# vani-nag/OWLRayTracing

Hardware: AMD Instinct MI355X
Metric: kNN queries/sec (10M pts, k=10) (higher is better)
Workload: dtype f32; 1 GPU; TrueKNN on 10000000 uniform-random 3-D points (numpy default_rng(0), [0,1)^3), k=10, start radius 0.25*(k/n)^(1/3)=0.0025; BASELINE.json configs[1]; ranks=1, n_points_total=10000000, k=10, kernel=team_kernel, parallelism=1 GPU

## Files before the change

### owlraytracing_amd/csrc/team_args.h

```cpp
#pragma once
#include <stdint.h>

#include <algorithm>
#include <cstdlib>

#include "lbvh.h"
#include "owlknn.h"

#ifndef TKNN_DIAG_BUILD
#define TKNN_DIAG_BUILD 0
#endif

namespace owlmi {

constexpr int kTeamBlock = 64;
inline int grab_for(int64_t count, int blocks, int turns, int cap) {
  if (const char *g = getenv("TKNN_GRAB")) return std::max(1, atoi(g));
  return (int)std::max<int64_t>(1, std::min<int64_t>(cap, count / ((int64_t)std::max(1, blocks) * 4 * turns)));
}
#ifndef TKNN_NREG3
#define TKNN_NREG3 1
#endif
inline int nreg_for(int k) { return k <= 16 ? 1 : (k <= 32 ? 2 : (k <= 48 && TKNN_NREG3 ? 3 : 4)); }

struct TeamArgs {
  LbvhView bvh, halo;
  LbvhWideView wide[2];
  float start_radius;
  const float *start_radii;
  int k;
  int max_rounds;
  int allow_unfinished;
  int first_step;
  int first_ext;
  float tie_span;
  int diag;
  int32_t ngroups;
  int32_t *out_idx;
  float *out_dist;
  int64_t *out_isect;
  tknnNeigh *out_fb;
  int32_t *out_level;
  uint8_t *done;
  int64_t *isect_sorted;
  int32_t *next_level;
  uint8_t *tie;
  int32_t *tie_list;
  const uint8_t *skip;
  int32_t skip_is;
  const int32_t *slot_count;
  int grab;
  const int32_t *row_slot;
  unsigned long long *counters;
};

}
```

### owlraytracing_amd/csrc/trueknn_team.hip

```cpp
#include "knn_thresholds.h"
#include "team_args.h"
#include "team_lanes.h"
#include "team_walk.h"
#include "trueknn_engine.h"

#include <algorithm>
#include <cmath>
#include <cstdio>
#include <cstdlib>
#include <cstring>

namespace owlmi {

namespace {

#ifndef TKNN_MAX_BLOCKS_3
#define TKNN_MAX_BLOCKS_3 256
#endif
#ifndef TKNN_MAX_BLOCKS_4
#define TKNN_MAX_BLOCKS_4 512
#endif
constexpr int max_blocks(int nreg) { return nreg == 4 ? TKNN_MAX_BLOCKS_4 : (nreg == 3 ? TKNN_MAX_BLOCKS_3 : 256); }
#ifndef TKNN_MAX_PER_QUERY
#define TKNN_MAX_PER_QUERY 72
#endif
#ifndef TKNN_MAX_PER_QUERY_2
#define TKNN_MAX_PER_QUERY_2 88
#endif
#ifndef TKNN_MAX_PER_QUERY_3
#define TKNN_MAX_PER_QUERY_3 88
#endif
#ifndef TKNN_MAX_PER_QUERY_4
#define TKNN_MAX_PER_QUERY_4 124
#endif
constexpr int max_per_query(int nreg) {
  return nreg == 1 ? TKNN_MAX_PER_QUERY : (nreg == 4 ? TKNN_MAX_PER_QUERY_4 : (nreg == 3 ? TKNN_MAX_PER_QUERY_3 : TKNN_MAX_PER_QUERY_2));
}
inline int lds_workgroups_per_cu(size_t lds) {
  const size_t granule = 1280, total = 160 * 1024;
  return lds ? (int)((total / granule) / ((lds + granule - 1) / granule)) : 1 << 20;
}
#ifndef TKNN_SORT_FIRST
#define TKNN_SORT_FIRST 1
#endif
#ifndef TKNN_TEAM_WAVES
#define TKNN_TEAM_WAVES 4
#endif
constexpr int kXcdCounter = kDbStats, kXcdCounterStride = 32;
constexpr int kTeamStack = 192;
constexpr int kQrecStride = 6;
constexpr int kScanBudget = 16384;
constexpr int kMaxStep = 2;
constexpr int kLdsQrec = 64 * kQrecStride * 4;
constexpr int kLdsCnt = 64 * 2 * 4;
constexpr int kLdsList = 64 * 4 + 16;
constexpr int kLdsStack = kTeamStack * 4;
constexpr int kLdsShared = (kLdsCnt + kLdsList) > kLdsStack ? (kLdsCnt + kLdsList) : kLdsStack;
constexpr int kLdsSharedPadded = (kLdsShared + 15) & ~15;
constexpr int kCandCap = kCandCapacity;
template <int NREG>
struct TeamLayout {
  static constexpr int kMaxPerQuery = max_per_query(NREG);
  static constexpr int kMaxBlocks = max_blocks(NREG);
  static constexpr int kLdsBlk = kMaxBlocks * 4;
  static constexpr int kLdsMask = 64 * kMaxPerQuery;
  static constexpr int kHiWords = kMaxBlocks > 256 ? (kMaxPerQuery + 31) / 32 : 0;
  static constexpr int kLdsHi = 64 * kHiWords * 4;
  static constexpr int kEntStride = kMaxPerQuery + 4;
  static constexpr int kLdsEnt = 4 * kEntStride * 4;
  static constexpr int kLdsCand = 4 * kCandCap * 8;
  static constexpr int kOffMask = kLdsQrec + kLdsBlk;
  static constexpr int kOffHi = kOffMask + kLdsMask;
  static constexpr int kOffShared = kOffHi + kLdsHi;
  static constexpr int kOffEnt = kOffShared + kLdsSharedPadded;
  static constexpr int kOffCand = kOffEnt + kLdsEnt;
  static constexpr int kTeamLds = kOffCand + kLdsCand;
  static_assert(kEntStride % 4 == 0 && kOffEnt % 16 == 0, "entry lists must be 16-byte aligned");
  static_assert(kLdsMask % 4 == 0, "the ninth bits are words");
  static_assert(kMaxPerQuery <= 124 && kMaxPerQuery / 4 < 32, "list-length buckets of the pass lists are one bit each of a 32-bit word");
};

struct TeamLds {
  float *qrec;
  int32_t *blk;
  uint8_t *qblk;
  uint32_t *qhi;
  uint32_t *qcnt;
  int32_t *qlist;
  int32_t *ent;
  unsigned long long *cand;
};

template <bool SELECT, bool HALO, int NREG, bool FULL, bool TWO>
__device__ __forceinline__ void team_pass(const TeamArgs &a, const TeamLds &L, int n_list, int32_t first_slot,
                                          const LbvhPoint *own_pts, const LbvhPoint *halo_pts, int lane) {
  const int team = lane >> 4, tl = lane & 15;
  constexpr int kMaxPerQuery = TeamLayout<NREG>::kMaxPerQuery, kEntStride = TeamLayout<NREG>::kEntStride;
  static_assert(!(SELECT && TWO), "only a COUNT pass serves two levels");
  n_list = __builtin_amdgcn_readfirstlane(n_list);
  [[maybe_unused]] unsigned long long tp[4] = {0, 0, 0, 0};
  for (int r0 = 0; r0 < n_list; r0 += 4) {
    [[maybe_unused]] unsigned long long tp_mark = 0;
    if (TKNN_DIAG_BUILD && (a.diag & 128)) tp_mark = __builtin_amdgcn_s_memtime();
#define TP_LAP(i)                                                     \
  do {                                                                \
    if (TKNN_DIAG_BUILD && (a.diag & 128)) {                          \
      const unsigned long long now_ = __builtin_amdgcn_s_memtime();   \
      tp[i] += now_ - tp_mark;                                        \
      tp_mark = now_;                                                 \
    }                                                                 \
  } while (0)
    const bool on = r0 + team < n_list;
    int qi = 0;
    if (on) qi = L.qlist[r0 + team];
    const float *rec = L.qrec + qi * kQrecStride;
    const float t_qx = rec[0], t_qy = rec[1], t_qz = rec[2];
    const int32_t t_qid = __float_as_int(rec[3]);
    const float t_r = rec[4];
    const float t_mg = (fmaxf(fmaxf(fabsf(t_qx), fabsf(t_qy)), fabsf(t_qz)) + 2.0f * t_r) * 4.76837158203125e-07f;
    const float in_below = t_r - t_mg, in_upto = t_r + t_mg;
    const float r_inner = t_r * 0.5f;
    const float i0_below = r_inner - t_mg, i0_upto = r_inner + t_mg;
    uint32_t cnt_i0 = 0;
    const int packed = __float_as_int(rec[5]);
    [[maybe_unused]] int32_t out_row = 0;
    if (SELECT) out_row = a.bvh.prim_id[first_slot + qi];
    const int my_n = on ? (packed & 0xff) : 0;
    const int steps = max(max((int)__builtin_amdgcn_readlane(my_n, 0), (int)__builtin_amdgcn_readlane(my_n, 16)),
                          max((int)__builtin_amdgcn_readlane(my_n, 32), (int)__builtin_amdgcn_readlane(my_n, 48)));
    if (TKNN_DIAG_BUILD && (a.diag & 16) && lane == 0) atomicAdd(&a.counters[15], (unsigned long long)steps);
    const uint8_t *mine = L.qblk + qi * kMaxPerQuery;
    const int last = my_n - 1;
    const int32_t nan_block = a.wide[0].count[0];
    const int own_pos = (packed >> 8) & 0xff;
    const int n_near = (packed >> 16) & 0xff;
    const int last_near = n_near ? n_near - 1 : last;
    const int both = min(own_pos, last_near - own_pos);
    const bool right_longer = last_near - own_pos > own_pos;
    auto list_pos = [&](int it) -> int {
      if (!SELECT) return it;
      const int half = (it + 1) >> 1;
      const int alt = (it & 1) ? half : -half;
      const int far = it - both;
      const int off = it <= 2 * both ? alt : (right_longer ? far : -far);
      return it > last_near ? it : own_pos + off;
    };
    auto list_entry = [&](int pos) -> int32_t {
      int lp = list_pos(pos);
      if (n_near && lp >= n_near) lp = kMaxPerQuery - 1 - (lp - n_near);
      const int at = min(max(lp, 0), kMaxPerQuery - 1);
      int slot_at = mine[at];
      if (TeamLayout<NREG>::kHiWords) slot_at |= (int)((L.qhi[qi * TeamLayout<NREG>::kHiWords + (at >> 5)] >> (at & 31)) & 1u) << 8;
      int32_t e = L.blk[slot_at];
      if (TKNN_DIAG_BUILD && (a.diag & 64)) e = L.blk[mine[0]];
      return resolve_entry<HALO>(pos <= last ? e : nan_block);
    };
    const int steps4 = (steps + 3) & ~3;
    int32_t *my_ent = L.ent + team * kEntStride;
    for (int base = 0; base < steps4 + 4; base += 16)
      if (base + tl < kEntStride) my_ent[base + tl] = list_entry(base + tl);
    t_wave_sync();
    uint32_t cnt = 0;
    uint32_t bd[NREG], bi[NREG];
#pragma unroll
    for (int j = 0; j < NREG; j++) {
      bd[j] = 0x7f7fffffu;
      bi[j] = 0u;
    }
    constexpr bool full = FULL;
    uint32_t left_out = 0xffffffffu;
    auto kth_dist = [&]() -> float {
      uint32_t reg = bd[0];
#pragma unroll
      for (int j = 1; j < NREG; j++) reg = ((a.k - 1) >> 4) == j ? bd[j] : reg;
      return __uint_as_float(t_lane_read(reg, (team << 4) + ((a.k - 1) & 15)));
    };
    float tau2 = INFINITY;
    bool dirty = false;
    uint32_t fill_n = 0;
    auto merge_buffer = [&]() {
      t_wave_sync();
      t_merge_rows<NREG>(bd, bi, left_out, full, L.cand + team * kCandCap, fill_n, tl);
      t_wave_sync();
      fill_n = 0;
      dirty = false;
      tau2 = knn_gate_from_worst(kth_dist());
    };
    auto in_box = [&](const LbvhPoint &p, float t, float radius, float below, float upto) -> unsigned long long {
      unsigned long long in_m = __ballot(t <= below);
      const unsigned long long maybe = __ballot(t <= upto);
      if (__builtin_expect(maybe != in_m, 0)) in_m |= maybe & __ballot(knn_in_box(p.x, p.y, p.z, radius, t_qx, t_qy, t_qz));
      return in_m;
    };
    auto process = [&](const LbvhPoint &p, bool own_block = false) {
      const float dx = p.x - t_qx, dy = p.y - t_qy, dz = p.z - t_qz;
      const float t = fmaxf(fmaxf(fabsf(dx), fabsf(dy)), fabsf(dz));
      const unsigned long long in_m = in_box(p, t, t_r, in_below, in_upto);
      cnt = t_count_keep(cnt, in_m, p.id);
      if (TWO) cnt_i0 = t_count(cnt_i0, in_box(p, t, r_inner, i0_below, i0_upto));
      if (SELECT) {
        const float d2 = t_dist2(dx, dy, dz);
        unsigned long long pm = in_m & __ballot(d2 <= tau2);
        if (own_block) pm &= __ballot(p.id != t_qid);
        if (TKNN_DIAG_BUILD && (a.diag & 1)) pm = 0;
        if (pm) {
          if (TKNN_DIAG_BUILD && (a.diag & 16) && lane == 0) atomicAdd(&a.counters[26], (unsigned long long)__popcll(pm));
          const uint32_t mine16 = (uint32_t)(pm >> (team << 4)) & 0xffffu;
          if ((mine16 >> tl) & 1u) {
            const unsigned long long key = ((unsigned long long)__float_as_uint(d2) << 32) | (uint32_t)p.id;
            L.cand[team * kCandCap + fill_n + __popc(mine16 & ((1u << tl) - 1u))] = key;
          }
          fill_n += __popc(mine16);
          dirty = true;
          if (__ballot(fill_n >= 16u) != 0ull) {
            if (TKNN_DIAG_BUILD && (a.diag & 16) && lane == 0) atomicAdd(&a.counters[27], 1ull);
            merge_buffer();
          }
        }
      }
    };
    const LbvhPoint *own_base = a.bvh.points;
    const uint32_t lane_bytes = (uint32_t)tl * (uint32_t)sizeof(LbvhPoint);
    typedef int32_t t_int4 __attribute__((ext_vector_type(4)));
    const t_int4 *my_groups = (const t_int4 *)my_ent;
    auto fetch = [&](int32_t entry) -> t_point4 {
      const LbvhPoint p = load_block_point<HALO>(own_pts, halo_pts, entry, own_base, lane_bytes);
      return t_point4{p.x, p.y, p.z, __int_as_float(p.id)};
    };
    auto unpack = [](const t_point4 &v) -> LbvhPoint { return LbvhPoint{v.x, v.y, v.z, __float_as_int(v.w)}; };
    auto sort_first = [&](const LbvhPoint &p) {
      const float dx = p.x - t_qx, dy = p.y - t_qy, dz = p.z - t_qz;
      const float t = fmaxf(fmaxf(fabsf(dx), fabsf(dy)), fabsf(dz));
      bool in = t <= t_r;
      if (__ballot(fabsf(t - t_r) <= t_mg) != 0ull) in = (t <= in_below) || ((t <= in_upto) && knn_in_box(p.x, p.y, p.z, t_r, t_qx, t_qy, t_qz));
      cnt = t_count(cnt, __ballot(in));
      bool cand = in && (p.id != t_qid);
      if (TKNN_DIAG_BUILD && (a.diag & 1)) cand = false;
      const uint32_t d2_bits = __float_as_uint(t_dist2(dx, dy, dz));
      unsigned long long *my_buf = L.cand + team * kCandCap;
      my_buf[tl] = ((unsigned long long)d2_bits << 32) | (uint32_t)p.id;
      t_wave_sync();
      t_sorted_row(d2_bits, (uint32_t)p.id, cand, tl, [&](int from) { return my_buf[from]; }, bd[0], bi[0]);
      t_wave_sync();
      tau2 = knn_gate_from_worst(kth_dist());
    };
    TP_LAP(0);
    t_point4 b0, b1, b2, b3;
    {
      const t_int4 g = my_groups[0];
      b0 = fetch(g.x);
      __builtin_amdgcn_sched_barrier(0);
      b1 = fetch(g.y);
      __builtin_amdgcn_sched_barrier(0);
      b2 = fetch(g.z);
      __builtin_amdgcn_sched_barrier(0);
      b3 = fetch(g.w);
      __builtin_amdgcn_sched_barrier(0);
    }
    for (int it = 0; it < steps; it += 4) {
      const t_int4 g = my_groups[(it >> 2) + 1];
      if (SELECT && it == 0) {
        if (NREG == 1 && TKNN_SORT_FIRST == 0)
          process(unpack(b0), true);
        else
          sort_first(unpack(b0));
      } else {
        process(unpack(b0));
      }
      b0 = fetch(g.x);
      process(unpack(b1));
      b1 = fetch(g.y);
      process(unpack(b2));
      b2 = fetch(g.z);
      process(unpack(b3));
      b3 = fetch(g.w);
      if (SELECT && dirty && __ballot(fill_n >= (uint32_t)TKNN_MERGE_AT) != 0ull) {
        if (TKNN_DIAG_BUILD && (a.diag & 16) && lane == 0) atomicAdd(&a.counters[27], 1ull);
        merge_buffer();
      }
      TP_LAP(it == 0 ? 1 : 2);
    }
    if (SELECT && dirty) {
      if (TKNN_DIAG_BUILD && (a.diag & 16) && lane == 0) atomicAdd(&a.counters[27], 1ull);
      merge_buffer();
    }
    if (SELECT && full) {
      uint32_t v = left_out;
      v = min(v, (uint32_t)__builtin_amdgcn_update_dpp(-1, (int)v, 0x128 , 0xf, 0xf, false));
      v = min(v, (uint32_t)__builtin_amdgcn_update_dpp(-1, (int)v, 0x124 , 0xf, 0xf, false));
      v = min(v, (uint32_t)__builtin_amdgcn_update_dpp(-1, (int)v, 0x122 , 0xf, 0xf, false));
      v = min(v, (uint32_t)__builtin_amdgcn_update_dpp(-1, (int)v, 0x121 , 0xf, 0xf, false));
      left_out = v;
    }
    cnt = t_team_sum(cnt);
    const uint32_t self = cnt ? 1u : 0u;
    const uint32_t others = cnt - self;
    if (TWO) cnt_i0 = t_team_sum(cnt_i0);
    uint32_t tied = 0u;
    if (SELECT) {
      bool tie[NREG];
      bool any = false;
#pragma unroll
      for (int j = 0; j < NREG; j++) {
        uint32_t before = t_team_shr1(bd[j]);
        if (j > 0) before |= t_dpp<0x121>(bd[j - 1]) & (tl == 0 ? 0xffffffffu : 0u);
        tie[j] = ((j > 0) | (tl >= 1)) & (16 * j + tl <= a.k) & (bd[j] == before);
        if (full && j == NREG - 1) tie[j] |= (tl == 15) & (left_out == bd[j]);
        any |= tie[j];
      }
      if (__ballot(any) != 0ull) {
        const float qmax = fmaxf(fmaxf(fabsf(t_qx), fabsf(t_qy)), fabsf(t_qz));
        any = false;
        bool edge = false;
        const float q_r0 = a.start_radii ? a.start_radii[a.bvh.prim_id[first_slot + qi]] : a.start_radius;
#pragma unroll
        for (int j = 0; j < NREG; j++) {
          const bool t = tie[j] && tie_may_straddle(__uint_as_float(bd[j]), q_r0, t_r, qmax, a.tie_span);
          any |= t;
          edge |= t && (16 * j + tl == a.k || (full && j == NREG - 1 && tl == 15 && left_out == bd[j]));
        }
        if (on && edge) knn_note_tie_edge(a.tie, first_slot + qi);
      }
      tied = ((uint32_t)(__ballot(any) >> (team * 16)) & 0xffffu) ? 1u : 0u;
    }
    if (on && tl == 0) {
      uint32_t *out = L.qcnt + qi * 2;
      if (!TWO) {
        out[0] = cnt;
        out[1] = (self << 31) | (tied << 30);
      } else {
        out[0] = cnt_i0;
        out[1] = cnt | (self << 31);
      }
    }
    if (SELECT) {
      if (on && others >= (uint32_t)a.k) {
#pragma unroll
        for (int reg = 0; reg < NREG; reg++) {
          const int j = tl + 16 * reg;
          if (j >= a.k) continue;
          const int64_t o = (int64_t)out_row * a.k + j;
          const int32_t prim = knn_key_prim(((uint64_t)bd[reg] << 32) | bi[reg]);
          const float d = __uint_as_float(bd[reg]);
          if (a.out_idx) a.out_idx[o] = prim;
          if (a.out_dist) a.out_dist[o] = d;
          if (a.out_fb) {
            int2 *rec8 = (int2 *)(a.out_fb + o);
            rec8[0] = make_int2(prim, __float_as_int(d));
            rec8[1] = make_int2(j == 0 ? 0 : a.k, 0);
            if (j != 0) rec8[2] = make_int2(0, 0);
          }
        }
      }
    }
    TP_LAP(3);
  }
#undef TP_LAP
  if (TKNN_DIAG_BUILD && (a.diag & 128) && lane == 0)
    for (int i = 0; i < 4; i++) atomicAdd(&a.counters[(SELECT ? 36 : 28) + i], tp[i]);
}

template <bool HALO, int NREG, bool FULL>
__global__ void __launch_bounds__(kTeamBlock) __attribute__((amdgpu_waves_per_eu(TKNN_TEAM_WAVES))) team_kernel(TeamArgs a) {
  extern __shared__ __align__(16) unsigned char smem[];
  const int lane = threadIdx.x & 63;
  const int wid = threadIdx.x >> 6;
  const int tl = lane & 15;
  using Lay = TeamLayout<NREG>;
  constexpr int kMaxPerQuery = Lay::kMaxPerQuery;
  unsigned char *base = smem + wid * Lay::kTeamLds;
  float *qrec = (float *)base;
  int32_t *blk = (int32_t *)(base + kLdsQrec);
  uint8_t *qblk = (uint8_t *)(base + Lay::kOffMask);
  uint32_t *qhi = (uint32_t *)(base + Lay::kOffHi);
  constexpr int kMaxBlocks = Lay::kMaxBlocks;
  uint32_t *qcnt = (uint32_t *)(base + Lay::kOffShared);
  int32_t *qlist = (int32_t *)(base + Lay::kOffShared + kLdsCnt);
  int32_t *stack = (int32_t *)(base + Lay::kOffShared);
  int32_t *ent = (int32_t *)(base + Lay::kOffEnt);
  unsigned long long *cand = (unsigned long long *)(base + Lay::kOffCand);

  const LbvhPoint *own_pts = a.bvh.points + tl, *halo_pts = a.halo.points ? a.halo.points + tl : a.bvh.points + tl;
  unsigned long long my_isect_sum = 0, wave_node_tests = 0, wave_point_tests = 0;
  uint32_t my_levels = 0, my_unfinished = 0;
  int wave_levels = 0, wave_err = 0;
  uint32_t my_handed = 0;
  [[maybe_unused]] unsigned long long diag_scanned = 0, diag_listed = 0;
  int wave_min_handover = 0x7fffffff;
#if TKNN_DIAG_BUILD
  unsigned long long ph[5] = {0, 0, 0, 0, 0}, t_mark = __builtin_amdgcn_s_memtime();
#define PHASE_END(i)                                         \
  do {                                                       \
    const unsigned long long now_ = __builtin_amdgcn_s_memtime(); \
    ph[i] += now_ - t_mark;                                  \
    t_mark = now_;                                           \
  } while (0)
#else
#define PHASE_END(i) \
  do {               \
  } while (0)
#endif

  const int xcc = (int)__builtin_amdgcn_s_getreg(6164 ) & 7;
  const int chunk = max(1, min(1024, a.ngroups / 128));
  uint32_t seg_empty = 0;
  for (;;) {
    int g = -1;
    for (int t = 0; t < 8 && g < 0; t++) {
      const int x = (xcc + t) & 7;
      if (seg_empty & (1u << x)) continue;
      int v = 0;
      if (lane == 0) v = (int)atomicAdd(&a.counters[kXcdCounter + kXcdCounterStride * x], 1ull);
      v = __builtin_amdgcn_readfirstlane(v);
      const int cand = ((v / chunk) * 8 + x) * chunk + (v % chunk);
      if (cand < a.ngroups)
        g = cand;
      else
        seg_empty |= 1u << x;
    }
    if (g < 0 || wave_err) break;

    const int32_t slot = g * 64 + lane;
    bool active = slot < a.bvh.n;
    if (a.skip) {
      if (active && (int32_t)a.skip[slot] == a.skip_is) active = false;
      if (__ballot(active) == 0ull) continue;
    }
    LbvhPoint q = {0.f, 0.f, 0.f, -1};
    if (active) q = a.bvh.points[slot];
    const int32_t row = active ? a.bvh.prim_id[slot] : 0;
    float r = a.start_radius;
    if (a.start_radii && active) r = a.start_radii[row];
    int level = 0;
    int64_t isect = 0;
    uint32_t prev_others = 0;
    int step = a.first_step;
    TeamLds L;
    L.qrec = qrec;
    L.blk = blk;
    L.qblk = qblk;
    L.qhi = qhi;
    L.qcnt = qcnt;
    L.qlist = qlist;
    L.ent = ent;
    L.cand = cand;

    bool reuse = false;
    int ext_next = a.first_ext;
    bool ext_ok = a.first_ext >= 0;
    for (;;) {
      PHASE_END(4);
      level = __builtin_amdgcn_readfirstlane(level);
      step = __builtin_amdgcn_readfirstlane(step);
      if (!a.start_radii) r = __uint_as_float(__builtin_amdgcn_readfirstlane(__float_as_uint(r)));
      int m = step < 1 ? 1 : (step > kMaxStep ? kMaxStep : step);
      if (reuse) m = 1;
      if (level + m > a.max_rounds) m = a.max_rounds - level;
      const float r_in0 = r;
      float r_out = r;
      for (int j = 1; j < m; j++) r_out = r_out * 2.0f;
      {
        float *rec = qrec + lane * kQrecStride;
        rec[0] = q.x;
        rec[1] = q.y;
        rec[2] = q.z;
        rec[3] = __int_as_float(q.id);
        rec[4] = r_out;
      }
      int my_nblk = 0;
      int n_in = 0, n_out = 0;
      int my_own_pos = 0;
      bool too_big = false;
      bool ext = !reuse && ext_next > 0 && level + m < a.max_rounds;
      ext = __builtin_amdgcn_readfirstlane((int)ext) != 0;
      if (reuse) {
        const int pk = __float_as_int(qrec[lane * kQrecStride + 5]);
        n_in = pk & 0xff;
        my_own_pos = (pk >> 8) & 0xff;
        n_out = (pk >> 24) & 0xff;
        my_nblk = n_in + n_out;
        reuse = false;
      } else
      for (;;) {
      const float r_walk = ext ? r_out * 2.0f : r_out;
      float lo_x = INFINITY, lo_y = INFINITY, lo_z = INFINITY, hi_x = -INFINITY, hi_y = -INFINITY, hi_z = -INFINITY;
      float reach_walk = -INFINITY, reach_step = -INFINITY;
      {
        const float qabs = fmaxf(fmaxf(fabsf(q.x), fabsf(q.y)), fabsf(q.z));
        const float mg = (qabs + 2.0f * r_walk) * 4.76837158203125e-07f;
        if (active && q.x == q.x) {
          lo_x = (q.x - r_walk) - 2.0f * mg;
          lo_y = (q.y - r_walk) - 2.0f * mg;
          lo_z = (q.z - r_walk) - 2.0f * mg;
          hi_x = (q.x + r_walk) + 2.0f * mg;
          hi_y = (q.y + r_walk) + 2.0f * mg;
          hi_z = (q.z + r_walk) + 2.0f * mg;
          reach_walk = r_walk + 2.0f * mg;
          reach_step = ext ? r_out + 2.0f * ((qabs + 2.0f * r_out) * 4.76837158203125e-07f) : reach_walk;
        }
      }
      float s_lo_x[4], s_lo_y[4], s_lo_z[4], s_hi_x[4], s_hi_y[4], s_hi_z[4];
      {
        const float r_lo_x = t_team_min(lo_x), r_lo_y = t_team_min(lo_y), r_lo_z = t_team_min(lo_z);
        const float r_hi_x = t_team_max(hi_x), r_hi_y = t_team_max(hi_y), r_hi_z = t_team_max(hi_z);
#pragma unroll
        for (int j = 0; j < 4; j++) {
          s_lo_x[j] = t_bcast(r_lo_x, 16 * j);
          s_lo_y[j] = t_bcast(r_lo_y, 16 * j);
          s_lo_z[j] = t_bcast(r_lo_z, 16 * j);
          s_hi_x[j] = t_bcast(r_hi_x, 16 * j);
          s_hi_y[j] = t_bcast(r_hi_y, 16 * j);
          s_hi_z[j] = t_bcast(r_hi_z, 16 * j);
        }
      }
      auto separation = [](float b_lo_x, float b_lo_y, float b_lo_z, float b_hi_x, float b_hi_y, float b_hi_z, float q_lo_x, float q_lo_y,
                           float q_lo_z, float q_hi_x, float q_hi_y, float q_hi_z) -> float {
        const float sx = fmaxf(b_lo_x - q_hi_x, q_lo_x - b_hi_x), sy = fmaxf(b_lo_y - q_hi_y, q_lo_y - b_hi_y),
                    sz = fmaxf(b_lo_z - q_hi_z, q_lo_z - b_hi_z);
        return fmaxf(fmaxf(sx, sy), sz);
      };
      auto overlaps_packet = [&](const LbvhBox &bx) -> bool {
        float best = INFINITY;
#pragma unroll
        for (int j = 0; j < 4; j++)
          best = fminf(best, separation(bx.lo[0], bx.lo[1], bx.lo[2], bx.hi[0], bx.hi[1], bx.hi[2], s_lo_x[j], s_lo_y[j], s_lo_z[j], s_hi_x[j],
                                        s_hi_y[j], s_hi_z[j]));
        return best <= 0.f;
      };
      float *node_boxes = (float *)ent;
      static_assert(64 * 6 * 4 <= Lay::kLdsEnt + Lay::kLdsCand, "the gather's child boxes borrow the entry lists' LDS");
      auto stash_boxes = [&](const LbvhBox &bx) {
        float2 *dst = (float2 *)(node_boxes + 6 * lane);
        dst[0] = make_float2(bx.lo[0], bx.lo[1]);
        dst[1] = make_float2(bx.lo[2], bx.hi[0]);
        dst[2] = make_float2(bx.hi[1], bx.hi[2]);
        t_wave_sync();
      };
      auto gap_to_me = [&](int src) -> float {
        int boff;
        asm("s_mul_i32 %0, %1, 24" : "=s"(boff) : "s"(src));
        const float2 *b = (const float2 *)((const char *)node_boxes + boff);
        const float2 b0 = b[0], b1 = b[1], b2 = b[2];
        return separation(b0.x, b0.y, b1.x, b1.y, b2.x, b2.y, q.x, q.y, q.z, q.x, q.y, q.z);
      };

      PHASE_END(0);
      my_own_pos = 0;
      int cur = 0;
      uint8_t *my_list = qblk + lane * kMaxPerQuery;
      if (Lay::kHiWords) {
#pragma unroll
        for (int w = 0; w < Lay::kHiWords; w++) qhi[lane * Lay::kHiWords + w] = 0u;
      }
      int nb = 0, scanned = 0;
      for (int tree = 0; tree < 2 && !too_big; tree++) {
        const LbvhWideView &wv = a.wide[tree];
        const int32_t tree_n = tree == 0 ? a.bvh.n : a.halo.n;
        if (tree_n <= 0 || wv.levels <= 0) continue;
        int sp = 0, nleaf = 0;
        if (lane == 0) stack[wv.levels > 1 ? 0 : kTeamStack - 1] = (wv.levels << 26) | 0;
        if (wv.levels > 1)
          sp = 1;
        else
          nleaf = 1;
        t_wave_sync();
        const int32_t last_block = wv.count[0] - 1;
        while ((sp > 0 || nleaf > 0) && !too_big) {
          if (sp > 0 && sp + nleaf + 63 <= kTeamStack) {
            const int32_t e = __builtin_amdgcn_readfirstlane(stack[sp - 1]);
            sp--;
            const int lvl = (e >> 26) - 1;
            const int32_t first_child = (e & 0x3ffffff) * 64;
            const int32_t c = first_child + lane;
            const bool valid = lvl == wv.levels - 1 ? (lane < wv.count[lvl] && first_child == 0) : (c < wv.count[lvl]);
            LbvhBox bx = {{0.f, 0.f, 0.f}, {0.f, 0.f, 0.f}};
            if (valid) bx = wv.level[lvl][c];
            wave_node_tests += 64;
            const bool ov = valid & overlaps_packet(bx);
            const unsigned long long om = __ballot(ov);
            const int cnt = __popcll(om);
            if (lvl > 1) {
              if (ov) stack[sp + t_rank(om)] = (lvl << 26) | c;
              sp += cnt;
            } else {
              unsigned long long rest = om;
              if (rest) stash_boxes(bx);
              while (rest) {
                const int src = 63 - __builtin_clzll(rest);
                rest &= ~(1ull << src);
                if (__ballot(gap_to_me(src) <= reach_walk) == 0ull) continue;
                if (lane == 0) stack[kTeamStack - 1 - nleaf] = (lvl << 26) | (first_child + src);
                nleaf++;
              }
            }
            t_wave_sync();
            continue;
          }
          if (nleaf == 0) {
            too_big = true;
            break;
          }
          auto leaf_boxes = [&](int i) -> LbvhBox {
            const int32_t e = __builtin_amdgcn_readfirstlane(stack[kTeamStack - nleaf + (i < nleaf ? i : nleaf - 1)]);
            return wv.level[0][min((e & 0x3ffffff) * 64 + lane, last_block)];
          };
          LbvhBox bx_next = leaf_boxes(0);
          for (int i = 0; i < nleaf && !too_big; i++) {
            const int32_t e = __builtin_amdgcn_readfirstlane(stack[kTeamStack - nleaf + i]);
            const int32_t first_child = (e & 0x3ffffff) * 64;
            const LbvhBox bx = bx_next;
            bx_next = leaf_boxes(i + 1);
            const bool valid = first_child + lane <= last_block;
            wave_node_tests += 64;
            const bool ov = valid & overlaps_packet(bx);
            unsigned long long om = __ballot(ov);
            scanned += __popcll(om);
            if (TKNN_DIAG_BUILD && (a.diag & 32)) diag_scanned += __popcll(om);
            if (scanned > kScanBudget) {
              too_big = true;
              break;
            }
            if (om) stash_boxes(bx);
            while (om) {
              const int src = __ffsll((long long)om) - 1;
              om &= om - 1;
              const float gap = gap_to_me(src);
              bool need = gap <= reach_walk;
              if (TKNN_DIAG_BUILD && (a.diag & 8)) need = false;
              if (__ballot(need) == 0ull) continue;
              if (nb >= kMaxBlocks) {
                too_big = true;
                break;
              }
              const int32_t block = first_child + src;
              blk[nb] = (int32_t)((uint32_t)block | ((uint32_t)tree << 31));
              if (tree == 0 && (uint32_t)(block - g * 4) < 4u && block == (slot >> 4)) my_own_pos = cur & 0xffff;
              if (need) {
                const bool inner = gap <= reach_step;
                const int at = inner ? (cur & 0xffff) : kMaxPerQuery - 1 - (cur >> 16);
                const int at_c = min(max(at, 0), kMaxPerQuery - 1);
                my_list[at_c] = (uint8_t)nb;
                if (Lay::kHiWords && nb >= 256) qhi[lane * Lay::kHiWords + (at_c >> 5)] |= 1u << (at_c & 31);
                cur += inner ? 1 : 0x10000;
              }
              nb++;
            }
          }
          nleaf = 0;
          t_wave_sync();
        }
        t_wave_sync();
      }
      if (TKNN_DIAG_BUILD && (a.diag & 32)) diag_listed += nb;
      n_in = cur & 0xffff, n_out = cur >> 16;
      if (ext) {
        if (too_big || __ballot(n_in + n_out > kMaxPerQuery) != 0ull) {
          ext = false;
          ext_ok = false;
          too_big = false;
          t_wave_sync();
          continue;
        }
        reuse = __ballot(active) != 0ull;
      }
      my_nblk = n_in;
      if (!ext) n_out = 0;
      break;
      }
      if (NREG < 3) {
        if (__ballot(my_nblk > kMaxPerQuery) != 0ull) too_big = true;
        if (too_big) {
          if (active) {
            a.done[slot] = 0;
            a.isect_sorted[slot] = isect;
            a.next_level[slot] = level;
            my_handed++;
          }
          wave_min_handover = min(wave_min_handover, level);
          active = false;
          break;
        }
      } else if (too_big || __ballot(my_nblk > kMaxPerQuery) != 0ull) {
        const bool hand_over = active && (too_big || my_nblk > kMaxPerQuery);
        if (hand_over) {
          a.done[slot] = 0;
          a.isect_sorted[slot] = isect;
          a.next_level[slot] = level;
          my_handed++;
          active = false;
        }
        wave_min_handover = min(wave_min_handover, level);
        if (__ballot(active) == 0ull) break;
      }
      const int my_packed = my_nblk | (my_own_pos << 8) | (my_nblk > n_in ? n_in << 16 : n_out << 24);
      qrec[lane * kQrecStride + 5] = __int_as_float(my_packed);

      PHASE_END(1);
      const bool speculate = m == 1 && active && level > 0 && prev_others * 8u >= (uint32_t)(a.k + a.k / 2);
      const bool count_first = active && !speculate;
      auto build_qlist = [&](bool sel) -> int {
        const int bucket = my_nblk >> 2;
        if (lane == 0) qlist[64] = 0;
        t_wave_sync();
        if (sel) __hip_atomic_fetch_or((uint32_t *)&qlist[64], 1u << bucket, __ATOMIC_RELAXED, __HIP_MEMORY_SCOPE_WAVEFRONT);
        t_wave_sync();
        uint32_t present = (uint32_t)__builtin_amdgcn_readfirstlane(qlist[64]);
        int base = 0, pos = 0;
        while (present) {
          const int b = __ffs((int)present) - 1;
          present &= present - 1u;
          const bool mine = sel && bucket == b;
          const unsigned long long bm = __ballot(mine);
          if (mine) pos = base + t_rank(bm);
          base += __popcll(bm);
        }
        if (sel) qlist[pos] = lane;
        t_wave_sync();
        return base;
      };
      {
        const int n_count = build_qlist(count_first);
        if (!(TKNN_DIAG_BUILD && (a.diag & 4))) {
          if (m > 1)
            team_pass<false, HALO, NREG, false, true>(a, L, n_count, g * 64, own_pts, halo_pts, lane);
          else
            team_pass<false, HALO, NREG, false, false>(a, L, n_count, g * 64, own_pts, halo_pts, lane);
        }
        t_wave_sync();
      }
      PHASE_END(2);
      uint32_t c0 = 0, c1 = 0, selfc = 0;
      int fin_at = -1;
      if (count_first) {
        c0 = qcnt[lane * 2 + 0];
        const uint32_t w1 = qcnt[lane * 2 + 1];
        c1 = m > 1 ? (w1 & 0x3fffffffu) : 0u;
        selfc = w1 >> 31;
        if (c0 - selfc >= (uint32_t)a.k)
          fin_at = 0;
        else if (m > 1 && c1 - selfc >= (uint32_t)a.k)
          fin_at = 1;
      }
      const bool select_now = speculate || fin_at >= 0;
      if (m > 1 && fin_at == 0) qrec[lane * kQrecStride + 4] = r_in0;
      {
        t_wave_sync();
        const int n_select = build_qlist(select_now);
        if (!(TKNN_DIAG_BUILD && (a.diag & 2))) team_pass<true, HALO, NREG, FULL, false>(a, L, n_select, g * 64, own_pts, halo_pts, lane);
        t_wave_sync();
      }
      PHASE_END(3);
      bool finished = fin_at >= 0;
      uint32_t last_others = 0;
      if (speculate) {
        c0 = qcnt[lane * 2 + 0];
        selfc = qcnt[lane * 2 + 1] >> 31;
        finished = c0 - selfc >= (uint32_t)a.k;
        fin_at = finished ? 0 : -1;
      }
      int levels_run = 0;
      if (active) {
        levels_run = finished ? fin_at + 1 : m;
        isect += c0;
        if (levels_run > 1) isect += c1;
        my_levels += (uint32_t)levels_run;
        last_others = (m > 1 ? c1 : c0) - selfc;
        prev_others = last_others;
      }
      wave_levels = max(wave_levels, (int)t_wave_max((float)(active ? level + levels_run : 0)));
      {
        const unsigned long long passes = (count_first ? 1ull : 0ull) + (select_now ? 1ull : 0ull);
        wave_point_tests += t_wave_sum(active ? (unsigned long long)my_nblk * LBVH_BLOCK * passes : 0ull);
      }
      if (finished) {
        my_isect_sum += (unsigned long long)isect;
        if (a.out_isect) a.out_isect[row] = isect;
        if (a.out_fb) a.out_fb[(int64_t)row * a.k].intersections = isect;
        const int fin_level = level + (fin_at > 0 ? fin_at : 0);
        if (a.out_level) a.out_level[row] = fin_level;
        if ((qcnt[lane * 2 + 1] >> 30) & 1u) knn_flag_tie(a.tie, a.tie_list, a.counters, slot, fin_level, 2);
      }
      active = active && !finished;
      level += m;
      t_wave_sync();
      if (__ballot(active) == 0ull) break;
      if (level >= a.max_rounds) {
        if (!a.allow_unfinished) wave_err |= 1;
        break;
      }
      for (int j = 0; j < m; j++) r = r * 2.0f;
      {
        const float pmax = t_wave_max(active ? (float)last_others : 0.f);
        float expect = pmax * 8.f;
        step = 1;
        while (step < kMaxStep && expect < 0.5f * (float)a.k) {
          step++;
          expect *= 8.f;
        }
        ext_next = ext_ok && expect < 2.5f * (float)a.k ? 1 : 0;
      }
    }
    if (active) my_unfinished++;
  }

  const unsigned long long isum = t_wave_sum(my_isect_sum), lsum = t_wave_sum((unsigned long long)my_levels), usum = t_wave_sum((unsigned long long)my_unfinished),
                           hsum = t_wave_sum((unsigned long long)my_handed);
  if (lane == 0) {
    unsigned long long *st = a.counters + kStatBase + (blockIdx.x & (kStatStripes - 1)) * kStatStride;
    atomicMax(&st[1], (unsigned long long)wave_levels);
    atomicAdd(&st[2], wave_node_tests);
    atomicAdd(&st[3], wave_point_tests);
    atomicAdd(&st[4], isum);
    atomicAdd(&st[6], lsum);
    if (usum) atomicAdd(&st[7], usum);
    if (hsum) {
      atomicAdd(&st[8], hsum);
      atomicMin(&st[9], (unsigned long long)wave_min_handover);
    }
    if (wave_err) atomicOr(&st[5], (unsigned long long)wave_err);
#if TKNN_DIAG_BUILD
    for (int i = 0; i < 5; i++) atomicAdd(&a.counters[10 + i], ph[i]);
    if (a.diag & 32) {
      atomicAdd(&a.counters[24], diag_scanned);
      atomicAdd(&a.counters[25], diag_listed);
    }
#endif
  }
}


__global__ void __launch_bounds__(256) team_prep_kernel(uint8_t *done, uint8_t *tie, int64_t n, unsigned long long *counters, int32_t *levels) {
  const int64_t tid = (int64_t)blockIdx.x * blockDim.x + threadIdx.x, nth = (int64_t)gridDim.x * blockDim.x;
  if (tid < kCounters + 8 * kXcdCounterStride) counters[tid] = tid == 9 ? ~0ull : 0ull;
  if (tid < kStatStripes * kStatStride) counters[kStatBase + tid] = (tid & (kStatStride - 1)) == 9 ? ~0ull : 0ull;
  const int64_t words = n / 16;
  uint4 *d16 = reinterpret_cast<uint4 *>(done), *t16 = reinterpret_cast<uint4 *>(tie);
  const uint4 ones = make_uint4(0x01010101u, 0x01010101u, 0x01010101u, 0x01010101u), zeros = make_uint4(0u, 0u, 0u, 0u);
  for (int64_t i = tid; i < words; i += nth) {
    d16[i] = ones;
    t16[i] = zeros;
  }
  for (int64_t i = words * 16 + tid; i < n; i += nth) {
    done[i] = 1;
    tie[i] = 0;
  }
  if (levels)
    for (int64_t i = tid; i < n; i += nth) levels[i] = -1;
}

}

bool Engine::team_kernel_supports(int k) { return k >= 1 && k <= 64; }


int Engine::first_step_estimate(const SolveArgs &sa) const {
  float radius = sa.start_radius;
  for (int m = 1; m < 3; m++) {
    if (expected_box_population(radius) >= 0.5 * sa.k) return m;
    radius *= 2.0f;
  }
  return 3;
}

bool Engine::solve_team(const SolveArgs &sa, tknnSolveInfo *info, hipStream_t s) {
  const int64_t n = bvh_.size();
  if (n >= (1ll << 28)) return false;
  TeamArgs a = team_args(sa);
  set_solve_args(a, sa);
  a.first_step = sa.d_start_radii ? 1 : first_step_estimate(sa);
  {
    float radius = sa.start_radius;
    for (int t = 1; t < std::min(a.first_step, kMaxStep); t++) radius *= 2.0f;
    a.first_ext = !sa.d_start_radii && expected_box_population(radius) < 2.5 * sa.k ? 1 : 0;
    if (const char *e = getenv("TKNN_TEAM_EXT")) a.first_ext = atoi(e) > 0 ? a.first_ext : -1;
  }
  {
    int dims = 0;
    for (int ax = 0; ax < 3; ax++) dims += scene_[3 + ax] > scene_[ax] ? 1 : 0;
    if (halo_count() > 0) dims = 3;
    a.tie_span = dims >= 3 ? 1.73206f : (dims == 2 ? 1.41422f : 1.00001f);
  }
  if (TKNN_DIAG_BUILD)
    if (const char *d = getenv("TKNN_TEAM_DIAG")) a.diag = atoi(d);
  a.ngroups = (int32_t)((n + 63) / 64);

  const int nreg = nreg_for(sa.k);
  const char *walk_all = getenv("TKNN_TEAM_WALK_ALL");
  if (sa.k > 32 && walk_all && atoi(walk_all)) {
    reset_solve_state(sa.d_levels, s);
    const tknnSolveInfo all = walk(sa, a, 4, nullptr, (int32_t)n, 0, false, s);
    if (info) *info = all;
    return true;
  }
  int per_cu = 2;
  static_assert(kDbStripes * kDbStripeWords >= 8 * kXcdCounterStride, "the packet counters borrow the words of RT-DBSCAN's striped statistics");
  const size_t lds = (size_t)kTeamBlock / 64 * (size_t)(nreg == 1 ? TeamLayout<1>::kTeamLds : (nreg == 2 ? TeamLayout<2>::kTeamLds
                                                         : (nreg == 3 ? TeamLayout<3>::kTeamLds : TeamLayout<4>::kTeamLds)));
  const bool full_list = sa.k == 16 * nreg;
  using TeamEntry = void (*)(TeamArgs);
  static const TeamEntry entries[2][4][2] = {
      {{team_kernel<false, 1, false>, team_kernel<false, 1, true>}, {team_kernel<false, 2, false>, team_kernel<false, 2, true>},
       {team_kernel<false, 3, false>, team_kernel<false, 3, true>}, {team_kernel<false, 4, false>, team_kernel<false, 4, true>}},
      {{team_kernel<true, 1, false>, team_kernel<true, 1, true>}, {team_kernel<true, 2, false>, team_kernel<true, 2, true>},
       {team_kernel<true, 3, false>, team_kernel<true, 3, true>}, {team_kernel<true, 4, false>, team_kernel<true, 4, true>}}};
  const TeamEntry entry = entries[halo_count() > 0 ? 1 : 0][nreg - 1][full_list ? 1 : 0];
  if (hipOccupancyMaxActiveBlocksPerMultiprocessor(&per_cu, (const void *)entry, kTeamBlock, lds) != hipSuccess) per_cu = 2;
  per_cu = std::max(1, std::min(per_cu, lds_workgroups_per_cu(lds)));
  if (const char *cap = getenv("TKNN_TEAM_WAVES_PER_CU"))
    per_cu = std::max(1, std::min(per_cu, atoi(cap)));
  const int64_t want = (a.ngroups + kTeamBlock / 64 - 1) / (kTeamBlock / 64);
  const int blocks = (int)std::max<int64_t>(1, std::min<int64_t>(want, (int64_t)cu_count_ * per_cu));

  hipLaunchKernelGGL(team_prep_kernel, dim3(cu_count_ * 4), dim3(256), 0, s, done_, tie_, n, counters_, sa.phase >= 2 ? nullptr : sa.d_levels);
  OWLMI_HIP(hipEventRecord(ev_a_, s));
  {
    void *kargs[] = {(void *)&a};
    OWLMI_HIP(hipLaunchKernel((const void *)entry, dim3(blocks), dim3(kTeamBlock), kargs, lds, s));
  }
  OWLMI_HIP(hipGetLastError());
  OWLMI_HIP(hipEventRecord(ev_b_, s));
  launch_tie_fix(sa, tie_list_, -1, std::min(cu_count_ * 4, kTieListCap / 4), s);
  OWLMI_HIP(hipEventRecord(ev_c_, s));
  fetch_stat_stripes(s);
  OWLMI_HIP(hipMemcpyAsync(h_counters_ + 10, counters_ + kTieCounter, 3 * sizeof(unsigned long long), hipMemcpyDeviceToHost, s));
  OWLMI_HIP(hipStreamSynchronize(s));
  const KernelStats st = fold_stat_stripes(true);
  float ms = 0;
  OWLMI_HIP(hipEventElapsedTime(&ms, ev_a_, ev_b_));
  if (st.handed_over == 0 && h_counters_[10] <= (unsigned long long)kTieListCap) {
    ties_early_ = true;
    early_tie_rows_ = (int64_t)h_counters_[10];
    early_tie_left_ = (int64_t)h_counters_[12];
    OWLMI_HIP(hipEventElapsedTime(&early_tie_ms_, ev_b_, ev_c_));
  }
#if TKNN_DIAG_BUILD
  if (getenv("TKNN_TEAM_DIAG")) {
    unsigned long long t[5];
    OWLMI_HIP(hipMemcpy(t, counters_ + 10, sizeof t, hipMemcpyDeviceToHost));
    const double tot = (double)(t[0] + t[1] + t[2] + t[3] + t[4]);
    unsigned long long wave_steps = 0;
    OWLMI_HIP(hipMemcpy(&wave_steps, counters_ + 15, sizeof wave_steps, hipMemcpyDeviceToHost));
    fprintf(stderr, "[team diag] block steps: %.3g wave steps x 4 teams for %.3g listed blocks (lockstep efficiency %.1f%%)\n",
            (double)wave_steps, (double)st.point_tests / LBVH_BLOCK, 100.0 * ((double)st.point_tests / LBVH_BLOCK) / (4.0 * (double)wave_steps));
    if (a.diag & 16) {
      unsigned long long g[2];
      OWLMI_HIP(hipMemcpy(g, counters_ + 26, sizeof g, hipMemcpyDeviceToHost));
      fprintf(stderr, "[team diag] inserts: %.4g candidates passed the gate after the sorted first block (%.2f per query), in %.4g lock-step rounds of the wave (%.2f per query)\n",
              (double)g[0], (double)g[0] / (double)n, (double)g[1], (double)g[1] / (double)n);
    }
    if (a.diag & 128) {
      unsigned long long g[12];
      OWLMI_HIP(hipMemcpy(g, counters_ + 28, sizeof g, hipMemcpyDeviceToHost));
      for (int pass = 0; pass < 2; pass++) {
        const unsigned long long *t4 = g + 8 * pass;
        const double tt = (double)(t4[0] + t4[1] + t4[2] + t4[3]);
        fprintf(stderr, "[team diag] %s pass, wave time: %.3g cycles in all; set-up %.1f%%  first group %.1f%%  other groups %.1f%%  epilogue %.1f%%\n",
                pass ? "SELECT" : "COUNT", tt, 100 * t4[0] / tt, 100 * t4[1] / tt, 100 * t4[2] / tt, 100 * t4[3] / tt);
      }
    }
    if (a.diag & 32) {
      unsigned long long g[2];
      OWLMI_HIP(hipMemcpy(g, counters_ + 24, sizeof g, hipMemcpyDeviceToHost));
      fprintf(stderr, "[team diag] gather: %.3g leaf blocks tested against the 64 queries, %.3g of them listed (%.1f%%)\n", (double)g[0], (double)g[1], 100.0 * (double)g[1] / (double)g[0]);
    }
    fprintf(stderr, "[team diag] mean busy time per wave %.2f ms of %.2f ms kernel time (%d waves; s_memtime at 100 MHz)\n",
            tot / 1e8 * 1e3 / blocks, ms, blocks);
    fprintf(stderr, "[team diag] wave-time shares: records %.1f%%  gather %.1f%%  count %.1f%%  select %.1f%%  rest %.1f%%\n",
            100 * t[0] / tot, 100 * t[1] / tot, 100 * t[2] / tot, 100 * t[3] / tot, 100 * t[4] / tot);
  }
#endif
  if (st.flags & 1ull) throw RoundsExceeded{};
  if (info) *info = solve_info(st, sa.start_radius, TKNN_KERNEL_TEAM, 16 * nreg, ms);
  const unsigned long long handed = st.handed_over;
  if (handed) {
    tknnSolveInfo tail;
    std::memset(&tail, 0, sizeof tail);
    const char *force = getenv("TKNN_TEAM_TAIL");
    const bool by_wave = !sa.d_start_radii && wave_kernel_available() &&
                         (force ? !strcmp(force, "wave") : (handed * 4ull >= (unsigned long long)n && sa.k <= 32));
    const bool by_walk = !by_wave && !(force && !strcmp(force, "lane"));
    const int first_handover_level = (int)st.first_handover_level;
    if (by_wave) {
      solve_wave(sa, &tail, s, true);
    } else if (by_walk) {
      compact_slots(false, s);
      tail = walk(sa, a, nreg, slot_list_, (int32_t)handed, first_handover_level, true, s);
    } else {
      if (sa.d_start_radii) throw ArgError{TKNN_E_UNSUPPORTED, "per-query start radii are served by the team kernels only (TKNN_TEAM_TAIL=lane)"};
      continue_lane(sa, first_handover_level, &tail, s);
    }
    if (getenv("TKNN_VERBOSE"))
      fprintf(stderr, "[team] %llu of %lld queries handed over from level %d on: team kernel %.2f ms, %s %.2f ms (%d launches)\n",
              handed, (long long)n, first_handover_level, ms, by_wave ? "wave kernel" : (by_walk ? "team walk" : "lane rounds"), tail.solve_ms,
              tail.dominant_kernel_launches);
    if (info) merge_tail(*info, tail, sa.start_radius, false);
  }
  return true;
}

}
```

Measured before the change: 1.983 billion queries/s.

## Merge extended-radius selection into the count round for reused-block queries

When a query is in reuse mode and its count pass shows enough neighbours are likely at the next doubled radius, it now runs the select pass directly at that doubled radius, using the packed in/out block counts to widen its block list. Such a query skips a separate count round and is marked as served, so the next iteration does not recount it. The level and radius advance by one extra step when every active lane took this path. The aim is to cut full count+select iterations per query. The cost is extra branching, more complex bookkeeping, and a larger select pass.

New measurement: 2.057 billion queries/s, median of 6. 1.04x the previous value.

```diff
diff --git a/owlraytracing_amd/csrc/team_args.h b/owlraytracing_amd/csrc/team_args.h
--- a/owlraytracing_amd/csrc/team_args.h
+++ b/owlraytracing_amd/csrc/team_args.h
@@ -33,6 +33,7 @@
   int allow_unfinished;
   int first_step;
   int first_ext;
+  int merge_ext;
   float tie_span;
   int diag;
   int32_t ngroups;
diff --git a/owlraytracing_amd/csrc/trueknn_team.hip b/owlraytracing_amd/csrc/trueknn_team.hip
--- a/owlraytracing_amd/csrc/trueknn_team.hip
+++ b/owlraytracing_amd/csrc/trueknn_team.hip
@@ -448,6 +448,7 @@
     bool reuse = false;
     int ext_next = a.first_ext;
     bool ext_ok = a.first_ext >= 0;
+    bool served = false;
     for (;;) {
       PHASE_END(4);
       level = __builtin_amdgcn_readfirstlane(level);
@@ -696,10 +697,11 @@
       qrec[lane * kQrecStride + 5] = __int_as_float(my_packed);
 
       PHASE_END(1);
-      const bool speculate = m == 1 && active && level > 0 && prev_others * 8u >= (uint32_t)(a.k + a.k / 2);
-      const bool count_first = active && !speculate;
-      auto build_qlist = [&](bool sel) -> int {
-        const int bucket = my_nblk >> 2;
+      const bool speculate = m == 1 && active && !served && level > 0 && prev_others * 8u >= (uint32_t)(a.k + a.k / 2);
+      const bool count_first = active && !served && !speculate;
+      served = false;
+      auto build_qlist = [&](bool sel, int nblk) -> int {
+        const int bucket = nblk >> 2;
         if (lane == 0) qlist[64] = 0;
         t_wave_sync();
         if (sel) __hip_atomic_fetch_or((uint32_t *)&qlist[64], 1u << bucket, __ATOMIC_RELAXED, __HIP_MEMORY_SCOPE_WAVEFRONT);
@@ -719,7 +721,7 @@
         return base;
       };
       {
-        const int n_count = build_qlist(count_first);
+        const int n_count = build_qlist(count_first, my_nblk);
         if (!(TKNN_DIAG_BUILD && (a.diag & 4))) {
           if (m > 1)
             team_pass<false, HALO, NREG, false, true>(a, L, n_count, g * 64, own_pts, halo_pts, lane);
@@ -741,36 +743,54 @@
         else if (m > 1 && c1 - selfc >= (uint32_t)a.k)
           fin_at = 1;
       }
+      int sel_nblk = my_nblk;
+      if (reuse && a.merge_ext && count_first && fin_at < 0 && ((m > 1 ? c1 : c0) - selfc) * 8u >= (uint32_t)(a.k + a.k / 2)) {
+        fin_at = m;
+        const int pk = __float_as_int(qrec[lane * kQrecStride + 5]);
+        sel_nblk = (pk & 0xff) + ((pk >> 24) & 0xff);
+        qrec[lane * kQrecStride + 4] = qrec[lane * kQrecStride + 4] * 2.0f;
+        qrec[lane * kQrecStride + 5] = __int_as_float(sel_nblk | (pk & 0xff00) | ((pk & 0xff) << 16) | (pk & (int)0xff000000u));
+      }
       const bool select_now = speculate || fin_at >= 0;
       if (m > 1 && fin_at == 0) qrec[lane * kQrecStride + 4] = r_in0;
       {
         t_wave_sync();
-        const int n_select = build_qlist(select_now);
+        const int n_select = build_qlist(select_now, sel_nblk);
         if (!(TKNN_DIAG_BUILD && (a.diag & 2))) team_pass<true, HALO, NREG, FULL, false>(a, L, n_select, g * 64, own_pts, halo_pts, lane);
         t_wave_sync();
       }
       PHASE_END(3);
-      bool finished = fin_at >= 0;
-      uint32_t last_others = 0;
+      const bool ext_sel = fin_at == m;
+      bool finished = fin_at >= 0 && !ext_sel;
+      uint32_t last_others = prev_others;
       if (speculate) {
         c0 = qcnt[lane * 2 + 0];
         selfc = qcnt[lane * 2 + 1] >> 31;
         finished = c0 - selfc >= (uint32_t)a.k;
         fin_at = finished ? 0 : -1;
       }
+      uint32_t c_ext = 0, n_back = 0;
+      if (ext_sel) {
+        c_ext = qcnt[lane * 2 + 0];
+        finished = c_ext - selfc >= (uint32_t)a.k;
+        const int pk = __float_as_int(qrec[lane * kQrecStride + 5]);
+        n_back = ((uint32_t)pk >> 24) & 0xffu;
+        qrec[lane * kQrecStride + 5] = __int_as_float(pk & 0x00ffffff);
+      }
       int levels_run = 0;
-      if (active) {
-        levels_run = finished ? fin_at + 1 : m;
+      if (count_first || speculate) {
+        levels_run = finished || ext_sel ? fin_at + 1 : m;
         isect += c0;
         if (levels_run > 1) isect += c1;
+        isect += c_ext;
         my_levels += (uint32_t)levels_run;
-        last_others = (m > 1 ? c1 : c0) - selfc;
+        last_others = ext_sel ? c_ext - selfc : (m > 1 ? c1 : c0) - selfc;
         prev_others = last_others;
       }
       wave_levels = max(wave_levels, (int)t_wave_max((float)(active ? level + levels_run : 0)));
       {
         const unsigned long long passes = (count_first ? 1ull : 0ull) + (select_now ? 1ull : 0ull);
-        wave_point_tests += t_wave_sum(active ? (unsigned long long)my_nblk * LBVH_BLOCK * passes : 0ull);
+        wave_point_tests += t_wave_sum(((unsigned long long)my_nblk * passes + n_back) * LBVH_BLOCK);
       }
       if (finished) {
         my_isect_sum += (unsigned long long)isect;
@@ -781,14 +801,23 @@
         if ((qcnt[lane * 2 + 1] >> 30) & 1u) knn_flag_tie(a.tie, a.tie_list, a.counters, slot, fin_level, 2);
       }
       active = active && !finished;
-      level += m;
+      int m_done = m;
+      if (reuse && a.merge_ext) {
+        if (__ballot(active && !ext_sel) == 0ull) {
+          m_done = m + 1;
+          reuse = false;
+        } else {
+          served = ext_sel;
+        }
+      }
+      level += m_done;
       t_wave_sync();
       if (__ballot(active) == 0ull) break;
       if (level >= a.max_rounds) {
         if (!a.allow_unfinished) wave_err |= 1;
         break;
       }
-      for (int j = 0; j < m; j++) r = r * 2.0f;
+      for (int j = 0; j < m_done; j++) r = r * 2.0f;
       {
         const float pmax = t_wave_max(active ? (float)last_others : 0.f);
         float expect = pmax * 8.f;
@@ -873,6 +902,8 @@
     for (int t = 1; t < std::min(a.first_step, kMaxStep); t++) radius *= 2.0f;
     a.first_ext = !sa.d_start_radii && expected_box_population(radius) < 2.5 * sa.k ? 1 : 0;
     if (const char *e = getenv("TKNN_TEAM_EXT")) a.first_ext = atoi(e) > 0 ? a.first_ext : -1;
+    a.merge_ext = 1;
+    if (const char *e = getenv("TKNN_TEAM_MERGE")) a.merge_ext = atoi(e) > 0 ? 1 : 0;
   }
   {
     int dims = 0;
```
